# 10183308/popsift

Hardware: AMD Instinct MI355X
Metric: Mpix/s SIFT extract on 1920x1080 (keypoints+descriptors) (higher is better)
Workload: dtype f32; 1 GPU; 1920x1080 u8 grayscale, default popsift::Config (2x upscale, 9 octaves, 3 levels, PopSift mode, loop descriptor, RootSift); distinct_images_per_gpu=16, contexts_per_gpu=3, images_per_launch=16

## Files before the change

### popsift_amd/csrc/ctx.hip

```cpp
#include <hip/hip_runtime.h>

#include <algorithm>
#include <cmath>
#include <cstdarg>
#include <cstddef>
#include <cstdio>
#include <cstdlib>
#include <cstring>
#include <new>
#include <vector>

#include "devfeatures.h"
#include "ext_list.h"
#include "kernels.h"
#include "sift_types.h"
#include "trace.h"

using namespace popsift_hip;

namespace {

constexpr int PITCH_ALIGN = 64;
constexpr int PROFILE_REPS = 4;

// ... 30 lines not shown
struct ImageSlot {
    DevBuf<char> input;
    void*        h_input = nullptr;
    size_t       h_input_cap = 0;
    DevBuf<float>       arena;
    DevBuf<InitExt>     iext;
    DevBuf<InitExt>     iext2;
    DevBuf<FilterState> fstate;
    DevBuf<int>         fhist;
    DevBuf<InitExt>     otmp;
    DevBuf<int>         orows;
    DevBuf<float>       sresp_in, sresp;
    DevBuf<StrongState> sstate;
    DevBuf<int>         schunk;
    DevBuf<Ext>         ext;
    DevBuf<float, PS_ORI_NBINS> ohist;
    DevBuf<popsift_hip_feature> feats;
    DevBuf<float, 128> desc;
    DevBuf<int>        map;
    DevBuf<float2>     rot;
    DevBuf<DescRec>    drec;
    DevBuf<int2>       cand;
    DevBuf<int>        partial;
    DevBuf<int>        ovf;
    bool               sized = false;
    DevBuf<popsift_hip_feature> alt_feats;
    DevBuf<float, 128>          alt_desc;
    bool moved = false;
    DevBuf<uint8_t, 128> desc_u8;
    bool u8_read = false;
    DevBuf<popsift_hip_frame>   frames;
    popsift_hip_frame*          h_frames = nullptr;
    DevBuf<int>                 fcounts, perm, inv;
    DevBuf<popsift_hip_feature> lfeats;
    int n_frames = 0;
    DevBuf<uint8_t> mask;
    void*           h_mask = nullptr;
    size_t          h_mask_cap = 0;

    size_t desc_cap() const { return std::min({desc.cap, map.cap, rot.cap, drec.cap}); }

    void release()
    {
        auto each = [](auto&... b) { ((void)b.release(), ...); };
        each(input, arena, iext, iext2, fstate, fhist, otmp, orows, sresp_in, sresp, sstate, schunk, ext, ohist, feats, desc, map, rot, drec, cand, partial, ovf, alt_feats,
             alt_desc, desc_u8, frames, fcounts, perm, inv, lfeats, mask);
        if (h_input) (void)hipHostFree(h_input);
        if (h_mask) (void)hipHostFree(h_mask);
        if (h_frames) (void)hipHostFree(h_frames);
    }
};

struct popsift_hip_ctx {
    int                device = 0;
    popsift_hip_params p{};
    int                levels = 3, L = 6;
    GaussRows<POPSIFT_HIP_MAX_LEVELS> tab{};
    GaussRows<POPSIFT_HIP_MAX_LEVELS> abs0{};
    float*             d_abs0 = nullptr;
    int                direct_path = 0;
// ... 238 lines not shown
    return hipMalloc(p, bytes);
}

template <class T, size_t PER>
int grow(popsift_hip_ctx* c, DevBuf<T, PER>& b, size_t need)
{
    if (need <= b.cap) return 0;
    HIP_TRY(c, b.release());
    HIP_TRY(c, ctx_malloc(c, (void**)&b.p, need * PER * sizeof(T)));
    b.cap = need;
    return 0;
}

void refresh_caps(popsift_hip_ctx* c)
{
    size_t cand = 1 << 30, desc = 1 << 30, hist = (size_t)1 << 40;
    for (int k = 0; k < c->nb; k++) {
        const ImageSlot& s = c->slot[k];
        cand = std::min(cand, s.cand.cap);
        desc = std::min(desc, s.desc_cap());
        hist = std::min(hist, s.ohist.cap);
        Slot& v = c->bd.s[k];
        v.arena = s.arena.p;
        v.ct = c->d_ct + k;
        v.cand = s.cand.p;
        v.ovf = s.ovf.p;
        v.iext = s.iext.p;
        v.iext2 = s.iext2.p;
        v.fstate = s.fstate.p;
        v.fhist = s.fhist.p;
        v.ohist = s.ohist.p;
        v.ext = s.ext.p;
        v.partial = s.partial.p;
        v.map = s.map.p;
        v.rot = s.rot.p;
        v.drec = s.drec.p;
        v.feats = s.feats.p;
        v.desc = s.desc.p;
    }
    c->cand_cap = (int)cand;
    c->desc_cap = (int)desc;
    c->ohist_cap = hist;
}

int slot_desc_cap(popsift_hip_ctx* c, ImageSlot& s, size_t need)
{
    if (need <= s.desc_cap()) return 0;
    HIP_TRY(c, s.desc.release());
    HIP_TRY(c, s.map.release());
    HIP_TRY(c, s.rot.release());
    HIP_TRY(c, s.drec.release());
    if (int rc = grow(c, s.desc, need)) return rc;
    if (int rc = grow(c, s.map, need)) return rc;
    if (int rc = grow(c, s.rot, need)) return rc;
    return grow(c, s.drec, need);
}

// ... 21 lines not shown
        c->frozen_octaves = plan.n_oct;

        c->in_w = c->in_h = 0;
        c->have_image = false;
        c->pd.n_oct = 0;
        c->ext_cap = 0;
        for (int k = 0; k < PS_MAX_BATCH; k++) c->slot[k].sized = false;

        pd = plan;
    } else {
        const OctDesc& last = pd.o[pd.n_oct - 1];
        total = pd.dog_fly ? (size_t)pd.o[0].dog_off + (size_t)pd.o[0].plane_stride
                           : (size_t)last.dog_off + (size_t)last.plane_stride * (size_t)(c->L - 1);
    }
    const size_t need_ext = (size_t)pd.n_oct * (size_t)c->sc.max_extrema;
    for (int k = 0; k < nb; k++) {
        ImageSlot& s = c->slot[k];
        if (s.sized) continue;
        if (int rc = grow(c, s.arena, total)) return rc;
        if (int rc = grow(c, s.iext, need_ext)) return rc;
        if (int rc = grow(c, s.ext, need_ext)) return rc;
        if (int rc = grow(c, s.feats, need_ext)) return rc;
        if (c->sc.filter_max > 0) {
            if (int rc = grow(c, s.iext2, need_ext)) return rc;
            if (int rc = grow(c, s.fstate, 1)) return rc;
            if (int rc = grow(c, s.fhist, filter_hist_bytes(c->sc.grid_size) / sizeof(int))) return rc;
        }
        if (c->p.feature_order == POPSIFT_HIP_ORDER_RASTER) {
            if (int rc = grow(c, s.otmp, need_ext)) return rc;
            if (int rc = grow(c, s.orows, order_rows(pd))) return rc;
        }
        if (int rc = grow(c, s.partial, (need_ext / scan_chunk() + 2) * scan_partials_per_chunk())) return rc;
        const int desc0 = c->desc_cap_init > 0 ? c->desc_cap_init
                                               : std::max(2 * c->sc.max_extrema, c->sc.max_extrema + c->sc.max_extrema / 4);
        if (int rc = slot_desc_cap(c, s, std::max(desc0, c->desc_cap))) return rc;
        int cand0 = std::max(c->cand_cap_init, DET_SUBQ);
        if (!c->cand_cap_user) {
            double px = 0;
            for (int o = 0; o < pd.n_oct; o++) px += (double)pd.o[o].w * pd.o[o].h;
            cand0 = std::max(cand0, (int)std::min(px / 8.0, 64.0 * 1024 * 1024));
        }
        if (int rc = grow(c, s.cand, std::max(cand0, c->cand_cap))) return rc;
        if (int rc = grow(c, s.ohist, std::max(c->ohist_cap_init > 0 ? (size_t)c->ohist_cap_init
                                                                      : std::min(need_ext, (size_t)2 * c->sc.max_extrema),
                                               c->slot[0].sized ? c->ohist_cap : (size_t)0)))
            return rc;
        if (int rc = grow(c, s.ovf, (size_t)pd.total_tiles + 1)) return rc;
        s.sized = true;
    }
    c->ext_cap = need_ext;
    if (!same) {
        *c->h_pd = pd;
        HIP_TRY(c, hipMemcpyAsync(c->d_pd, c->h_pd, sizeof(PyrDesc), hipMemcpyHostToDevice, c->stream));
        c->pd = pd;
        c->in_w = w;
        c->in_h = h;
        c->rep.num_octaves = pd.n_oct;
        c->rep.base_w = bw;
        c->rep.base_h = bh;
        double px = 0;
        for (int o = 0; o < pd.n_oct; o++) px += (double)pd.o[o].w * pd.o[o].h;
// ... 316 lines not shown
    }
    return launch_strongest(c->pd, c->d_pd, c->sc, c->batch_keep, sb, c->nb, c->stream);
}

int enqueue_descriptor_stages(popsift_hip_ctx* c, const BatchDesc& lb, bool filtered, bool with_ori, const FrameBatch* fb)
{
    const bool stages = (c->profile == 2);
    auto       mark = [&](int k) -> hipError_t { return stages ? hipEventRecord(c->ev_stage[k], c->stream) : hipSuccess; };
    HIP_TRY(c, mark(POPSIFT_HIP_STAGE_ORIENTATION));
    if (with_ori) {
        HIP_TRY(c, launch_orientation(c->d_pd, c->bd, c->nb, c->sc, filtered, (int)c->ohist_cap, c->kp_waves, c->stream));
        SYNC_CHK(c, "k_orientation");
    }
    HIP_TRY(c, mark(POPSIFT_HIP_STAGE_SCAN));
    const int n_chunks = std::max((int)(((size_t)c->pd.n_oct * c->sc.max_extrema + scan_chunk() - 1) / scan_chunk()), 1);
    if (with_ori)
        HIP_TRY(c, launch_scan(c->d_pd, lb, c->nb, c->sc, filtered, (int)c->ohist_cap, n_chunks, c->desc_cap, c->stream));
    else
        HIP_TRY(c, launch_scan_apply(c->d_pd, lb, c->nb, c->sc, n_chunks, c->desc_cap, c->stream));
    SYNC_CHK(c, "k_scan_local / k_scan_apply");
    HIP_TRY(c, mark(POPSIFT_HIP_STAGE_DESCRIPTOR));
    HIP_TRY(c, launch_descriptors(c->d_pd, c->bd, c->nb, c->sc, c->desc_cap, c->kp_waves, c->stream));
    SYNC_CHK(c, "descriptor kernel");
    if (fb) {
        HIP_TRY(c, launch_frame_out(c->bd, *fb, c->nb, c->desc_cap, c->frames_max, c->stream));
        SYNC_CHK(c, "k_frame_out");
    }
    HIP_TRY(c, mark(POPSIFT_HIP_STAGE_COUNT));
    HIP_TRY(c, hipMemcpyAsync(c->h_ct, c->d_ct, sizeof(Counters) * (size_t)c->nb, hipMemcpyDeviceToHost, c->stream));
    return 0;
}

int enqueue_keypoint_stages(popsift_hip_ctx* c, bool counters_cleared = false)
{
    POPSIFT_RANGE("popsift_hip: keypoint stages");
// ... 218 lines not shown
            ext_max = std::max(ext_max, ext_sum);
        }
        const bool desc_short = ori_max > c->desc_cap;
        const bool cand_short = qmax > c->cand_cap / DET_SUBQ;
        const bool hist_short = (size_t)ext_max > c->ohist_cap && !c->ori_given;
        if (!desc_short && !cand_short && !hist_short) {
            fits = true;
            break;
        }
        if (desc_short)
            if (int rc = ensure_cap(c, [&](ImageSlot& s) { return slot_desc_cap(c, s, ori_max + ori_max / 8 + 1024); }))
                return rc;
        if (cand_short)
            if (int rc = ensure_cap(c, [&](ImageSlot& s) { return grow(c, s.cand, DET_SUBQ * (qmax + qmax / 8 + 64)); }))
                return rc;
        if (hist_short) {
            const size_t need = (size_t)ext_max + (size_t)ext_max / 8 + 1024;
            if (int rc = ensure_cap(c, [&](ImageSlot& s) { return grow(c, s.ohist, need); })) return rc;
        }
        if (int rc = c->describe ? enqueue_describe_stages(c) : enqueue_keypoint_stages(c)) return rc;
        HIP_TRY(c, hipEventRecord(c->ev_end, c->stream));
        rerun = true;
    }
    if (!fits) return fail(c, POPSIFT_HIP_ERR_DEVICE, "the keypoint buffers still do not fit after 8 grow-and-rerun rounds");
    popsift_hip_report& r = c->rep;
    for (int k = 0; k < c->nb; k++) {
        c->n_feat[k] = c->describe ? c->slot[k].n_frames : c->h_ct[k].ext_total;
        c->n_desc[k] = std::min(c->h_ct[k].ori_total, c->desc_cap);
    }
    Counters& h0 = c->h_ct[0];
    int       next = h0.ori_total;
    for (int o = PS_MAX_OCT - 1; o >= 0; o--) {
        if (h0.ext_ct[o] > 0) {
            h0.ori_ct[o] = next - h0.ori_ps[o];
// ... 804 lines not shown
```

### popsift_amd/csrc/kernels.h

```cpp
#pragma once
#include <hip/hip_runtime.h>

#include <algorithm>

#include "sift_types.h"

namespace popsift_hip {

struct Taps {
    float g[PS_GA];
};

struct BlurArgs {
    int64_t src_off;
    int64_t dst_off;
    int64_t dog_off;
    int     w, h, pitch;
    int     tiles_x, tiles_y;
    int     in_w, in_h, in_pitch;
    float   shift;
    int     fast2x;
    Taps    taps;
    int64_t next0_off;
    int     next_pitch;
// ... 56 lines not shown
hipError_t launch_blur_octaves(const BlurArgs& base, int level, const PyrDesc* d_pd, const PyrDesc& pd, const BatchDesc& bd,
                               int nb, int halo, hipStream_t s);
hipError_t launch_blur_level0_sep(const BlurArgs& a, const Taps& vt, const BatchDesc& bd, int nb, int halo, int is_f32,
                                  hipStream_t s);
int        scale_tile_h();

hipError_t launch_dog_plane(float* dog, const float* upper, const float* lower, size_t n, hipStream_t s);
int        extrema_units(int w, int h);
hipError_t launch_extrema(const PyrDesc& pd, const PyrDesc* d_pd, const BatchDesc& bd, int nb, const SiftConsts& sc, int cand_cap,
                          bool filtered, hipStream_t s, hipEvent_t mid, const MaskArgs* ma);

hipError_t launch_orientation(const PyrDesc* d_pd, const BatchDesc& bd, int nb, const SiftConsts& sc, bool filtered, int hist_cap,
                              int blocks, hipStream_t s);
int        scan_chunk();
int        scan_partials_per_chunk();
hipError_t launch_scan(const PyrDesc* d_pd, const BatchDesc& bd, int nb, const SiftConsts& sc, bool filtered, int hist_cap,
                       int n_chunks, int desc_cap, hipStream_t s);
hipError_t launch_descriptors(const PyrDesc* d_pd, const BatchDesc& bd, int nb, const SiftConsts& sc, int desc_cap, int blocks,
                              hipStream_t s);

hipError_t launch_desc_modes(const PyrDesc* d_pd, const BatchDesc& bd, int nb, const SiftConsts& sc, int desc_cap, int blocks,
                             hipStream_t s);

hipError_t launch_scan_apply(const PyrDesc* d_pd, const BatchDesc& bd, int nb, const SiftConsts& sc, int n_chunks, int desc_cap,
                             hipStream_t s);

constexpr int FRAME_CHUNK = 256;
int        frame_chunks(int n_max);
hipError_t launch_frame_count(const PyrDesc* d_pd, const FrameBatch& fb, int nb, const SiftConsts& sc, int given, int n_max,
                              hipStream_t s);
hipError_t launch_frame_place(const PyrDesc* d_pd, const BatchDesc& bd, const FrameBatch& fb, int nb, const SiftConsts& sc,
                              int given, int n_max, hipStream_t s);
// ... 41 lines not shown
```

### popsift_amd/csrc/keypoint.hip

```cpp
#include <hip/hip_runtime.h>

#include "ext_list.h"
#include "kernels.h"
#include "keypoint_dev.h"
#include "sift_types.h"

namespace popsift_hip {
namespace {

constexpr float ORI_WINFACTOR = 1.5f;

struct Taps {
    const char* row;
    const char* dn;
    const char* up;
    __device__ __forceinline__ Taps(const float* layer, int pitch)
        : row((const char*)layer), dn((const char*)(layer + pitch)), up((const char*)(layer - pitch)) {}
    __device__ __forceinline__ void load_b(unsigned int b, float& xp, float& xm, float& yp, float& ym) const
    {
        xp = *(const float*)(row + (size_t)b + 4);
        xm = *(const float*)(row + (size_t)b - 4);
        yp = *(const float*)(dn + (size_t)b);
        ym = *(const float*)(up + (size_t)b);
    }
// ... 38 lines not shown
    const float d = (fabsf(x) + 1e-18f) + mod;
    const float t = y * __builtin_amdgcn_rcpf(d);
    const float s = t * t;
    float       p = fmaf(-0.02984253503382206f, s, 0.13406537473201752f);
    p = fmaf(p, s, -0.2964776158332825f);
    p = fmaf(p, s, 0.4928465187549591f);
    p = fmaf(p, s, -0.8470170497894287f);
    p = fmaf(p, s, 2.5464210510253906f);
    const float th = t * p;
    const float sg = copysignf(scale, x);
    return fmaf(th, sg, fmaf(-2.0f, sg, k0));
}

typedef __attribute__((address_space(3))) fix64 lds_fix64;
typedef __attribute__((address_space(3))) unsigned int lds_u32;
typedef __attribute__((address_space(3))) short lds_i16;
typedef __attribute__((address_space(3))) unsigned long long lds_u64;

#ifndef KP_NW
#define KP_NW 1
#endif
constexpr int ORI_COPIES = 4;

__global__ __launch_bounds__(64 * KP_NW) void k_orientation(const PyrDesc* __restrict__ pdp, BatchDesc bd, SiftConsts sc,
                                                     int filtered, int hist_cap)
{
    const float* __restrict__   arena = bd.s[blockIdx.y].arena;
    Counters* __restrict__      ct = bd.s[blockIdx.y].ct;
    const InitExt* __restrict__ iext = filtered ? bd.s[blockIdx.y].iext2 : bd.s[blockIdx.y].iext;
    float* __restrict__         ohist = bd.s[blockIdx.y].ohist;
    const int n_oct = pdp->n_oct, L = pdp->L;
    constexpr int    NB = PS_ORI_NBINS + 10;
    __shared__ fix64 s_hist[KP_NW][ORI_COPIES][NB];
    const int        wave = threadIdx.x >> 6, lane = threadIdx.x & 63;
    fix64*           hall = &s_hist[wave][0][0];
    fix64*           hist = s_hist[wave][lane & (ORI_COPIES - 1)];

    __shared__ int ps[PS_MAX_OCT + 1];
    const int total = min(ext_prefix(ps, ct, sc.max_extrema, n_oct), hist_cap);

    for (XcdSlice sl = xcd_slice<KP_NW>(); sl.more(total); sl.s += sl.step) {
        const int g = sl.index();
        if (g >= total) continue;
        const int o = uniform(ext_octave(ps, n_oct, g));
        const InitExt  ie = iext[(size_t)o * sc.max_extrema + (g - uniform(ps[o]))];
        const OctDesc* od = &pdp->o[o];
        const int      w = uniform(od->w), h = uniform(od->h), pitch = uniform(od->pitch);
        const int      lvl = uniform(min(max(ie.lpos, 0), L - 1));
        const float*   layer = arena + uniform64(od->data_off + lvl * od->plane_stride);

        for (int k = lane; k < ORI_COPIES * NB; k += 64) hall[k] = 0ull;
        wave_lds_sync();

        const float x = uniformf(ie.xpos), y = uniformf(ie.ypos), sig = uniformf(ie.sigma);
        const float sigw = ORI_WINFACTOR * sig;
        const int   rad = (int)roundf(3.0f * sigw);
        const float factor2 = (-0.5f / (sigw * sigw)) * 1.4426950408889634f;
        const int   sq_thres = rad * rad;
// ... 53 lines not shown
            bin(xb, yb, b0 - b1, b2 - b3, true);
        }
        if (t == 2) {
            coord(min(i + 64, loops - 1), xb, yb, ob);
            taps.load_b(ob, b0, b1, b2, b3);
        }
        if (t > 0) bin(xa, ya, a0 - a1, a2 - a3, i < loops);
        if (t == 2) bin(xb, yb, b0 - b1, b2 - b3, i + 64 < loops);
        wave_lds_sync();

        if (lane < PS_ORI_NBINS) {
            fix64 acc = 0ull;
#pragma unroll
            for (int k = 0; k < ORI_COPIES; k++)
                acc += hall[k * NB + lane] + (lane < NB - PS_ORI_NBINS ? hall[k * NB + PS_ORI_NBINS + lane] : 0ull);
            ohist[(size_t)g * PS_ORI_NBINS + lane] = from_fix(acc);
        }
        wave_lds_sync();
    }
}

__device__ __forceinline__ float quad_from_prev(float v)
{
    return __int_as_float(__builtin_amdgcn_update_dpp(0, __float_as_int(v), 0x93, 0xf, 0xf, false));
}
__device__ __forceinline__ float quad_from_next(float v)
{
    return __int_as_float(__builtin_amdgcn_update_dpp(0, __float_as_int(v), 0x39, 0xf, 0xf, false));
}
template <int CTRL>
__device__ __forceinline__ int quad_xchg(int v)
{
    return __builtin_amdgcn_update_dpp(0, v, CTRL, 0xf, 0xf, false);
}
__device__ __forceinline__ float div3(float x)
{
    const float r = 0.333333343267440796f;
    const float q = x * r;
    return fmaf(fmaf(-3.0f, q, x), r, q);
}

__device__ __forceinline__ int ori_peaks_quad(const float* __restrict__ hsrc, int j, bool have, float* angle_out)
{
    constexpr int N = PS_ORI_NBINS, M = N / 4;
    float         h[M], t[M];
#pragma unroll
    for (int b = 0; b < M; b++) h[b] = have ? hsrc[M * j + b] : 0.0f;
#pragma unroll
    for (int pass = 0; pass < 3; pass++) {
        {
            const float lft = quad_from_prev(h[M - 1]), rgt = quad_from_next(h[0]);
#pragma unroll
            for (int b = 0; b < M; b++) t[b] = div3(((b == 0 ? lft : h[b - 1]) + h[b]) + (b == M - 1 ? rgt : h[b + 1]));
        }
        {
            const float lft = quad_from_prev(t[M - 1]), rgt = quad_from_next(t[0]);
#pragma unroll
            for (int b = 0; b < M; b++) h[b] = div3(((b == 0 ? lft : t[b - 1]) + t[b]) + (b == M - 1 ? rgt : t[b + 1]));
        }
    }
    float refined[M], yval[M];
    {
        const float lft = quad_from_prev(h[M - 1]), rgt = quad_from_next(h[0]);
#pragma unroll
        for (int b = 0; b < M; b++) {
            const int   bin = M * j + b;
            const int   prev = (bin == 0) ? N - 1 : bin - 1;
            const float hp = (b == 0) ? lft : h[b - 1], hv = h[b], hn = (b == M - 1) ? rgt : h[b + 1];
            bool        predicate = hv > fmaxf(hp, hn);
            const float num = predicate ? 3.0f * hp - 4.0f * hv + 1.0f * hn : 0.0f;
            const float denB = predicate ? 2.0f * (hp - 2.0f * hv + hn) : 1.0f;
            const float newbin = num / denB;
            predicate = (predicate && newbin >= 0.0f && newbin <= 2.0f);
            refined[b] = predicate ? prev + newbin : -1.0f;
            yval[b] = predicate ? -(num * num) / (4.0f * denB) + hp : -INFINITY;
        }
    }
    unsigned int used = 0u;
    float        best0 = 0.0f;
    int          angles = 0;
#pragma unroll
    for (int k = 0; k < POPSIFT_HIP_ORI_MAX; k++) {
        float bv = 0.0f, br = -1.0f;
        int   bi = -1;
#pragma unroll
        for (int b = 0; b < M; b++) {
            const bool take = !((used >> b) & 1u) && (bi < 0 || yval[b] > bv);
            bv = take ? yval[b] : bv;
            br = take ? refined[b] : br;
            bi = take ? M * j + b : bi;
        }
        {
            const float ov = __int_as_float(quad_xchg<0xB1>(__float_as_int(bv))), orf = __int_as_float(quad_xchg<0xB1>(__float_as_int(br)));
            const int   oi = quad_xchg<0xB1>(bi);
            const bool  take = ov > bv || (ov == bv && oi < bi);
            bv = take ? ov : bv;
            br = take ? orf : br;
            bi = take ? oi : bi;
        }
        {
            const float ov = __int_as_float(quad_xchg<0x4E>(__float_as_int(bv))), orf = __int_as_float(quad_xchg<0x4E>(__float_as_int(br)));
            const int   oi = quad_xchg<0x4E>(bi);
            const bool  take = ov > bv || (ov == bv && oi < bi);
            bv = take ? ov : bv;
            br = take ? orf : br;
            bi = take ? oi : bi;
        }
        const int mine = bi - M * j;
        if (mine >= 0 && mine < M) used |= 1u << mine;
        if (k == 0) best0 = bv;
        if (bv >= 0.8f * best0) {
            float chosen_bin = br;
            if (chosen_bin >= N) chosen_bin -= N;
            angle_out[k] = fmaf(F_PI2 * chosen_bin, 1.0f / N, -F_PI);
            angles = k + 1;
        } else {
            angle_out[k] = 0.0f;
        }
    }
    return angles;
}

__device__ __forceinline__ DescRec make_desc_rec(const PyrDesc* __restrict__ pdp, const Ext& e, float angle, float cos_t, float sin_t)
{
    DescRec        r;
    const OctDesc* od = &pdp->o[e.octave];
    const int      lvl = min(max(e.lpos, 0), pdp->L - 1);
    const long long off = od->data_off + lvl * od->plane_stride;
    const float    x = e.xpos, y = e.ypos;
    const float    SBP = fabsf(DESC_MAGNIFY * e.sigma);
    const float    cell_px = (2.83f * SBP + 1.0f) * (2.83f * SBP + 1.0f);
    const int      fbits = min(max(31 - (int)ceilf(log2f(361.0f * cell_px)), 2), 14);
    const float    csbp = cos_t * SBP, ssbp = sin_t * SBP;
    const float    bsz = fabsf(csbp) + fabsf(ssbp);
    const float    ext_r = 2.5f * bsz;
// ... 8 lines not shown
    r.ang_bins = angle * (4.0f / F_PI);
    if (!(fabsf(r.ang_bins) <= 16.0f)) r.ang_bins = (float)remainder((double)angle * (4.0 / 3.14159265358979323846), 8.0);
    r.inv_c = (fabsf(r.crsbp) > 1e-20f) ? __builtin_amdgcn_rcpf(r.crsbp) : 0.0f;
    r.inv_s = (fabsf(r.srsbp) > 1e-20f) ? __builtin_amdgcn_rcpf(r.srsbp) : 0.0f;
    r.xymin = ((unsigned int)xmin & 0xffffu) | ((unsigned int)ymin << 16);
    r.xymax = ((unsigned int)xmax & 0xffffu) | ((unsigned int)ymax << 16);
    r.off_lo = (unsigned int)((unsigned long long)off & 0xffffffffull);
    r.off_hi = (unsigned int)((unsigned long long)off >> 32);
    r.misc = (unsigned int)od->pitch | ((unsigned int)fbits << 16) | ((SBP != 0.0f) ? (1u << 24) : 0u);
    return r;
}


constexpr int SCAN_ITEMS = 1;
constexpr int SCAN_CHUNK = 256 * SCAN_ITEMS;
constexpr int SCAN_LT = 256;
constexpr int SCAN_LCHUNK = SCAN_LT / 4;
constexpr int SCAN_SUB = SCAN_CHUNK / SCAN_LCHUNK;

__global__ __launch_bounds__(SCAN_LT) void k_scan_local(const PyrDesc* __restrict__ pdp, SiftConsts sc, BatchDesc bd,
                                                     int filtered, int hist_cap)
{
    const Counters* __restrict__ ct = bd.s[blockIdx.y].ct;
    const InitExt* __restrict__  iext = filtered ? bd.s[blockIdx.y].iext2 : bd.s[blockIdx.y].iext;
    const float* __restrict__    ohist = bd.s[blockIdx.y].ohist;
    Ext* __restrict__            ext = bd.s[blockIdx.y].ext;
    int* __restrict__            partial = bd.s[blockIdx.y].partial;
    static_assert(SCAN_CHUNK % SCAN_LCHUNK == 0 && SCAN_LT % 64 == 0, "four lanes per extremum, whole waves");
    __shared__ int s_wsum[SCAN_LT / 64];
    __shared__ int s_ps[PS_MAX_OCT + 1];
    const int      n_oct = pdp->n_oct;
    const int total = ext_prefix(s_ps, ct, sc.max_extrema, n_oct);
    const int tid = threadIdx.x;
    const int j = tid & 3;
    for (int chunk = blockIdx.x; chunk * SCAN_LCHUNK < total; chunk += gridDim.x) {
    const int  base = chunk * SCAN_LCHUNK;
    const int  g = base + (tid >> 2);
    const bool valid = g < total;
    const int  gc = min(g, total - 1);
    const int     o = ext_octave(s_ps, n_oct, gc);
    const InitExt ie = iext[(size_t)o * sc.max_extrema + (gc - s_ps[o])];
    Ext           e;
    e.xpos = ie.xpos;
    e.ypos = ie.ypos;
    e.lpos = ie.lpos;
    e.sigma = ie.sigma;
    e.octave = o;
    e.idx_ori = 0;
    const bool have = gc < hist_cap;
    const int  n = ori_peaks_quad(ohist + (size_t)min(gc, max(hist_cap - 1, 0)) * PS_ORI_NBINS, j, have, e.orientation);
    e.num_ori = have ? n : 0;
    if (!have)
        for (int q = 0; q < POPSIFT_HIP_ORI_MAX; q++) e.orientation[q] = 0.0f;
    const int self = (valid && j == 0) ? e.num_ori : 0;

    const WgScan scan = wg_scan<SCAN_LT / 64>(self, s_wsum);
    if (valid && j == 0) {
        e.idx_ori = scan.excl;
        ext[g] = e;
    }
    if (tid == SCAN_LT - 1) partial[chunk] = scan.excl + self;
    __syncthreads();
    }
}

__global__ __launch_bounds__(256) void k_scan_apply(const PyrDesc* __restrict__ pdp, SiftConsts sc, BatchDesc bd,
                                                    int with_drec, int desc_cap)
{
    Counters* __restrict__            ct = bd.s[blockIdx.y].ct;
    Ext* __restrict__                 ext = bd.s[blockIdx.y].ext;
    const int* __restrict__           partial = bd.s[blockIdx.y].partial;
    int* __restrict__                 map = bd.s[blockIdx.y].map;
    float2* __restrict__              rot = bd.s[blockIdx.y].rot;
    DescRec* __restrict__             drec = with_drec ? bd.s[blockIdx.y].drec : nullptr;
    popsift_hip_feature* __restrict__ feats = bd.s[blockIdx.y].feats;
    __shared__ int s_red[4];
    __shared__ int s_ps[PS_MAX_OCT + 1];
    const int      n_oct = pdp->n_oct;
    const int      tid = threadIdx.x, lane = tid & 63, wave = tid >> 6;
    const int total = ext_prefix(s_ps, ct, sc.max_extrema, n_oct);
    const int nb = (total + SCAN_CHUNK - 1) / SCAN_CHUNK;
    if (nb == 0 && blockIdx.x == 0 && tid == 0) {
        ct->ori_total = 0;
        ct->ext_total = 0;
        for (int o = 0; o < PS_MAX_OCT; o++) {
            ct->ext_ct[o] = 0;
            ct->ext_ps[o] = 0;
        }
    }
    for (int chunk = blockIdx.x; chunk < nb; chunk += gridDim.x) {
    const int base = chunk * SCAN_CHUNK;

    int acc = 0;
    for (int b = tid; b < chunk * SCAN_SUB; b += 256) acc += partial[b];
    acc = wave_sum(acc);
    if (lane == 0) s_red[wave] = acc;
    __syncthreads();
    const int chunk_offset = s_red[0] + s_red[1] + s_red[2] + s_red[3];
    int offset = chunk_offset;
    for (int k = 0; k < (tid * SCAN_ITEMS) / SCAN_LCHUNK; k++) offset += partial[chunk * SCAN_SUB + k];

    const int g0 = base + tid * SCAN_ITEMS;
#pragma unroll
    for (int k = 0; k < SCAN_ITEMS; k++) {
        const int g = g0 + k;
        if (g < total) {
            Ext       e = ext[g];
            const int idx = e.idx_ori + offset;
            const int n = e.num_ori;
            ext[g].idx_ori = idx;
            popsift_hip_feature f;
            const float         scl = powf(2.0f, (float)(e.octave - sc.up_fac_int));
            f.debug_octave = e.octave;
            f.xpos = e.xpos * scl;
            f.ypos = e.ypos * scl;
// ... 332 lines not shown
            const float rn = scalbnf(__builtin_amdgcn_rsqf(sq), sc.norm_multi);
            v0 = v0 * rn;
            v1 = v1 * rn;
        }
        desc[(size_t)d * 128 + lane] = v0;
        desc[(size_t)d * 128 + 64 + lane] = v1;
        wave_lds_sync();
    }
}

}

hipError_t launch_orientation(const PyrDesc* pd, const BatchDesc& bd, int nb, const SiftConsts& sc, bool filtered, int hist_cap,
                              int blocks, hipStream_t s)
{
    hipLaunchKernelGGL(k_orientation, dim3(blocks / KP_NW, nb), dim3(64 * KP_NW), 0, s, pd, bd, sc, filtered ? 1 : 0, hist_cap);
    return hipGetLastError();
}

hipError_t launch_scan(const PyrDesc* pd, const BatchDesc& bd, int nb, const SiftConsts& sc, bool filtered, int hist_cap,
                       int n_chunks, int desc_cap, hipStream_t s)
{
    hipLaunchKernelGGL(k_scan_local, dim3(std::min(n_chunks * SCAN_SUB, 512 * SCAN_SUB), nb), dim3(SCAN_LT), 0, s, pd, sc, bd,
                       filtered ? 1 : 0, hist_cap);
    return launch_scan_apply(pd, bd, nb, sc, n_chunks, desc_cap, s);
}

hipError_t launch_scan_apply(const PyrDesc* pd, const BatchDesc& bd, int nb, const SiftConsts& sc, int n_chunks, int desc_cap,
                             hipStream_t s)
{
    hipLaunchKernelGGL(k_scan_apply, dim3(std::min(n_chunks, 1024), nb), dim3(256), 0, s, pd, sc, bd,
                       sc.desc_mode == POPSIFT_HIP_DESC_LOOP ? 1 : 0, desc_cap);
    return hipGetLastError();
}

int scan_chunk() { return SCAN_CHUNK; }
int scan_partials_per_chunk() { return SCAN_SUB; }

hipError_t launch_descriptors(const PyrDesc* pd, const BatchDesc& bd, int nb, const SiftConsts& sc, int desc_cap, int blocks,
                              hipStream_t s)
// ... 10 lines not shown
```

### popsift_amd/csrc/keypoint_dev.h

```cpp
#pragma once
#include <hip/hip_runtime.h>

#include "wave_dev.h"

namespace popsift_hip {

constexpr float F_PI = 3.14159265358979323846f;
constexpr float F_PI2 = 2.0f * 3.14159265358979323846f;
constexpr float DESC_MAGNIFY = 3.0f;

typedef unsigned long long fix64;
__device__ __forceinline__ float from_fix(fix64 v) { return (float)((double)v * (1.0 / 1048576.0)); }

__device__ __forceinline__ void wave_lds_sync()
{
    __builtin_amdgcn_fence(__ATOMIC_SEQ_CST, "wavefront");
    __builtin_amdgcn_wave_barrier();
}

__device__ __forceinline__ float wave_allsum(float v)
{
#define PS_DPP_ADD(CTRL) v += __int_as_float(__builtin_amdgcn_update_dpp(0, __float_as_int(v), CTRL, 0xf, 0xf, false))
    PS_DPP_ADD(0xB1);
    PS_DPP_ADD(0x4E);
// ... 3 lines not shown
    const float r0 = __int_as_float(__builtin_amdgcn_readlane(__float_as_int(v), 0));
    const float r1 = __int_as_float(__builtin_amdgcn_readlane(__float_as_int(v), 16));
    const float r2 = __int_as_float(__builtin_amdgcn_readlane(__float_as_int(v), 32));
    const float r3 = __int_as_float(__builtin_amdgcn_readlane(__float_as_int(v), 48));
    return (r0 + r1) + (r2 + r3);
}

__device__ __forceinline__ float plane_at(const float* pl, int idx)
{
    return *(const float*)((const char*)pl + (size_t)((unsigned int)idx * 4u));
}

#ifndef KP_CHUNK
#define KP_CHUNK 256
#endif
struct XcdSlice {
    int x, s, step;
    __device__ __forceinline__ int index() const { return ((s / KP_CHUNK) * 8 + x) * KP_CHUNK + (s % KP_CHUNK); }
    __device__ __forceinline__ bool more(int total) const { return (s / KP_CHUNK) * 8 * KP_CHUNK < total; }
};
template <int NW>
__device__ __forceinline__ XcdSlice xcd_slice()
{
    XcdSlice sl;
    sl.x = blockIdx.x & 7;
    sl.s = (int)(blockIdx.x >> 3) * NW + uniform((int)(threadIdx.x >> 6));
    sl.step = (int)(gridDim.x >> 3) * NW;
    return sl;
}

__device__ __forceinline__ float div_nr(float a, float b)
{
    const float r = __builtin_amdgcn_rcpf(b);
    const float q = a * r;
    return fmaf(fmaf(-b, q, a), r, q);
}
__device__ __forceinline__ float atan2_acc(float y, float x)
{
    const float ax = fabsf(x), ay = fabsf(y);
// ... 16 lines not shown
```

### popsift_amd/csrc/sift_types.h

```cpp
#pragma once
#include <stdint.h>

#include <hip/hip_vector_types.h>

#include "../../include/popsift_hip.h"

#define PS_MAX_OCT POPSIFT_HIP_MAX_OCTAVES
#define PS_MAX_PLANES (POPSIFT_HIP_MAX_LEVELS + 3)
#define PS_GA POPSIFT_HIP_GAUSS_ALIGN
#define PS_ORI_NBINS 36

struct OctDesc {
    float*  data;
    float*  dog;
    int64_t data_off;
    int64_t dog_off;
    int64_t plane_stride;
    int     w, h, pitch;
    int     tile_begin;
};

struct PyrDesc {
    int     n_oct;
    int     levels;
// ... 62 lines not shown
};
#define DET_SUBQ 64

#define PS_MAX_BATCH POPSIFT_HIP_MAX_BATCH
struct FilterState;
struct Slot {
    float*               arena;
    Counters*            ct;
    const void*          input;
    int2*                cand;
    int*                 ovf;
    InitExt*             iext;
    InitExt*             iext2;
    FilterState*         fstate;
    int*                 fhist;
    float*               ohist;
    Ext*                 ext;
    int*                 partial;
    int*                 map;
    float2*              rot;
    DescRec*             drec;
    popsift_hip_feature* feats;
    float*               desc;
};
struct BatchDesc {
    Slot s[PS_MAX_BATCH];
};

#define FILTER_MAX_CELLS 4096
struct FilterState {
    int                active;
// ... 81 lines not shown
```

Before: 4011 Mpix/s.

## Fuse orientation peak finding and local scan into the orientation kernel

The orientation kernel now processes groups of 16 extrema per wave, keeps their histograms in LDS instead of writing them to a global ohist buffer, then runs the quad-lane peak search and a wave-level scan in the same kernel, writing Ext records and per-group partials. The separate k_scan_local kernel and the per-slot ohist allocation are removed, and scan_apply gains a vectorised partial sum plus a one-wave sub-chunk prefix in place of a serial loop. This saves a global round trip of histograms and one kernel launch. In exchange it uses more LDS per block and sets a launch-bounds occupancy hint, and the orientation grid is resized. The work per wave is also coarser, which may hurt load balance.

```diff
diff --git a/popsift_amd/csrc/ctx.hip b/popsift_amd/csrc/ctx.hip
--- a/popsift_amd/csrc/ctx.hip
+++ b/popsift_amd/csrc/ctx.hip
@@ -68,7 +68,6 @@
     DevBuf<StrongState> sstate;
     DevBuf<int>         schunk;
     DevBuf<Ext>         ext;
-    DevBuf<float, PS_ORI_NBINS> ohist;
     DevBuf<popsift_hip_feature> feats;
     DevBuf<float, 128> desc;
     DevBuf<int>        map;
@@ -97,7 +96,7 @@
     void release()
     {
         auto each = [](auto&... b) { ((void)b.release(), ...); };
-        each(input, arena, iext, iext2, fstate, fhist, otmp, orows, sresp_in, sresp, sstate, schunk, ext, ohist, feats, desc, map, rot, drec, cand, partial, ovf, alt_feats,
+        each(input, arena, iext, iext2, fstate, fhist, otmp, orows, sresp_in, sresp, sstate, schunk, ext, feats, desc, map, rot, drec, cand, partial, ovf, alt_feats,
              alt_desc, desc_u8, frames, fcounts, perm, inv, lfeats, mask);
         if (h_input) (void)hipHostFree(h_input);
         if (h_mask) (void)hipHostFree(h_mask);
@@ -366,12 +365,11 @@
 
 void refresh_caps(popsift_hip_ctx* c)
 {
-    size_t cand = 1 << 30, desc = 1 << 30, hist = (size_t)1 << 40;
+    size_t cand = 1 << 30, desc = 1 << 30;
     for (int k = 0; k < c->nb; k++) {
         const ImageSlot& s = c->slot[k];
         cand = std::min(cand, s.cand.cap);
         desc = std::min(desc, s.desc_cap());
-        hist = std::min(hist, s.ohist.cap);
         Slot& v = c->bd.s[k];
         v.arena = s.arena.p;
         v.ct = c->d_ct + k;
@@ -381,7 +379,6 @@
         v.iext2 = s.iext2.p;
         v.fstate = s.fstate.p;
         v.fhist = s.fhist.p;
-        v.ohist = s.ohist.p;
         v.ext = s.ext.p;
         v.partial = s.partial.p;
         v.map = s.map.p;
@@ -392,7 +389,6 @@
     }
     c->cand_cap = (int)cand;
     c->desc_cap = (int)desc;
-    c->ohist_cap = hist;
 }
 
 int slot_desc_cap(popsift_hip_ctx* c, ImageSlot& s, size_t need)
@@ -444,6 +440,8 @@
                            : (size_t)last.dog_off + (size_t)last.plane_stride * (size_t)(c->L - 1);
     }
     const size_t need_ext = (size_t)pd.n_oct * (size_t)c->sc.max_extrema;
+    c->ohist_cap = std::max(c->ohist_cap, c->ohist_cap_init > 0 ? (size_t)c->ohist_cap_init
+                                                                 : std::min(need_ext, (size_t)2 * c->sc.max_extrema));
     for (int k = 0; k < nb; k++) {
         ImageSlot& s = c->slot[k];
         if (s.sized) continue;
@@ -471,10 +469,6 @@
             cand0 = std::max(cand0, (int)std::min(px / 8.0, 64.0 * 1024 * 1024));
         }
         if (int rc = grow(c, s.cand, std::max(cand0, c->cand_cap))) return rc;
-        if (int rc = grow(c, s.ohist, std::max(c->ohist_cap_init > 0 ? (size_t)c->ohist_cap_init
-                                                                      : std::min(need_ext, (size_t)2 * c->sc.max_extrema),
-                                               c->slot[0].sized ? c->ohist_cap : (size_t)0)))
-            return rc;
         if (int rc = grow(c, s.ovf, (size_t)pd.total_tiles + 1)) return rc;
         s.sized = true;
     }
@@ -821,11 +815,8 @@
     }
     HIP_TRY(c, mark(POPSIFT_HIP_STAGE_SCAN));
     const int n_chunks = std::max((int)(((size_t)c->pd.n_oct * c->sc.max_extrema + scan_chunk() - 1) / scan_chunk()), 1);
-    if (with_ori)
-        HIP_TRY(c, launch_scan(c->d_pd, lb, c->nb, c->sc, filtered, (int)c->ohist_cap, n_chunks, c->desc_cap, c->stream));
-    else
-        HIP_TRY(c, launch_scan_apply(c->d_pd, lb, c->nb, c->sc, n_chunks, c->desc_cap, c->stream));
-    SYNC_CHK(c, "k_scan_local / k_scan_apply");
+    HIP_TRY(c, launch_scan_apply(c->d_pd, lb, c->nb, c->sc, n_chunks, c->desc_cap, c->stream));
+    SYNC_CHK(c, "k_scan_apply");
     HIP_TRY(c, mark(POPSIFT_HIP_STAGE_DESCRIPTOR));
     HIP_TRY(c, launch_descriptors(c->d_pd, c->bd, c->nb, c->sc, c->desc_cap, c->kp_waves, c->stream));
     SYNC_CHK(c, "descriptor kernel");
@@ -1074,10 +1065,7 @@
         if (cand_short)
             if (int rc = ensure_cap(c, [&](ImageSlot& s) { return grow(c, s.cand, DET_SUBQ * (qmax + qmax / 8 + 64)); }))
                 return rc;
-        if (hist_short) {
-            const size_t need = (size_t)ext_max + (size_t)ext_max / 8 + 1024;
-            if (int rc = ensure_cap(c, [&](ImageSlot& s) { return grow(c, s.ohist, need); })) return rc;
-        }
+        if (hist_short) c->ohist_cap = std::max(c->ohist_cap, (size_t)ext_max + (size_t)ext_max / 8 + 1024);
         if (int rc = c->describe ? enqueue_describe_stages(c) : enqueue_keypoint_stages(c)) return rc;
         HIP_TRY(c, hipEventRecord(c->ev_end, c->stream));
         rerun = true;
diff --git a/popsift_amd/csrc/kernels.h b/popsift_amd/csrc/kernels.h
--- a/popsift_amd/csrc/kernels.h
+++ b/popsift_amd/csrc/kernels.h
@@ -94,8 +94,6 @@
                               int blocks, hipStream_t s);
 int        scan_chunk();
 int        scan_partials_per_chunk();
-hipError_t launch_scan(const PyrDesc* d_pd, const BatchDesc& bd, int nb, const SiftConsts& sc, bool filtered, int hist_cap,
-                       int n_chunks, int desc_cap, hipStream_t s);
 hipError_t launch_descriptors(const PyrDesc* d_pd, const BatchDesc& bd, int nb, const SiftConsts& sc, int desc_cap, int blocks,
                               hipStream_t s);
 
diff --git a/popsift_amd/csrc/keypoint.hip b/popsift_amd/csrc/keypoint.hip
--- a/popsift_amd/csrc/keypoint.hip
+++ b/popsift_amd/csrc/keypoint.hip
@@ -76,6 +76,7 @@
 
 typedef __attribute__((address_space(3))) fix64 lds_fix64;
 typedef __attribute__((address_space(3))) unsigned int lds_u32;
+typedef __attribute__((address_space(3))) float lds_f32;
 typedef __attribute__((address_space(3))) short lds_i16;
 typedef __attribute__((address_space(3))) unsigned long long lds_u64;
 
@@ -84,13 +85,118 @@
 #endif
 constexpr int ORI_COPIES = 4;
 
-__global__ __launch_bounds__(64 * KP_NW) void k_orientation(const PyrDesc* __restrict__ pdp, BatchDesc bd, SiftConsts sc,
-                                                     int filtered, int hist_cap)
+__device__ __forceinline__ float div3(float x)
+{
+    const float r = 0.333333343267440796f;
+    const float q = x * r;
+    return fmaf(fmaf(-3.0f, q, x), r, q);
+}
+
+__device__ __forceinline__ float quad_from_prev(float v)
+{
+    return __int_as_float(__builtin_amdgcn_update_dpp(0, __float_as_int(v), 0x93, 0xf, 0xf, false));
+}
+__device__ __forceinline__ float quad_from_next(float v)
+{
+    return __int_as_float(__builtin_amdgcn_update_dpp(0, __float_as_int(v), 0x39, 0xf, 0xf, false));
+}
+template <int CTRL>
+__device__ __forceinline__ int quad_xchg(int v)
+{
+    return __builtin_amdgcn_update_dpp(0, v, CTRL, 0xf, 0xf, false);
+}
+
+__device__ __forceinline__ int ori_peaks_quad(const lds_f32* __restrict__ hsrc, int j, bool have, float* angle_out)
+{
+    constexpr int N = PS_ORI_NBINS, M = N / 4;
+    float         h[M], t[M];
+#pragma unroll
+    for (int b = 0; b < M; b++) h[b] = have ? hsrc[M * j + b] : 0.0f;
+#pragma unroll
+    for (int pass = 0; pass < 3; pass++) {
+        {
+            const float lft = quad_from_prev(h[M - 1]), rgt = quad_from_next(h[0]);
+#pragma unroll
+            for (int b = 0; b < M; b++) t[b] = div3(((b == 0 ? lft : h[b - 1]) + h[b]) + (b == M - 1 ? rgt : h[b + 1]));
+        }
+        {
+            const float lft = quad_from_prev(t[M - 1]), rgt = quad_from_next(t[0]);
+#pragma unroll
+            for (int b = 0; b < M; b++) h[b] = div3(((b == 0 ? lft : t[b - 1]) + t[b]) + (b == M - 1 ? rgt : t[b + 1]));
+        }
+    }
+    float refined[M], yval[M];
+    {
+        const float lft = quad_from_prev(h[M - 1]), rgt = quad_from_next(h[0]);
+#pragma unroll
+        for (int b = 0; b < M; b++) {
+            const int   bin = M * j + b;
+            const int   prev = (bin == 0) ? N - 1 : bin - 1;
+            const float hp = (b == 0) ? lft : h[b - 1], hv = h[b], hn = (b == M - 1) ? rgt : h[b + 1];
+            bool        predicate = hv > fmaxf(hp, hn);
+            const float num = predicate ? 3.0f * hp - 4.0f * hv + 1.0f * hn : 0.0f;
+            const float denB = predicate ? 2.0f * (hp - 2.0f * hv + hn) : 1.0f;
+            const float newbin = num / denB;
+            predicate = (predicate && newbin >= 0.0f && newbin <= 2.0f);
+            refined[b] = predicate ? prev + newbin : -1.0f;
+            yval[b] = predicate ? -(num * num) / (4.0f * denB) + hp : -INFINITY;
+        }
+    }
+    unsigned int used = 0u;
+    float        best0 = 0.0f;
+    int          angles = 0;
+#pragma unroll
+    for (int k = 0; k < POPSIFT_HIP_ORI_MAX; k++) {
+        float bv = 0.0f, br = -1.0f;
+        int   bi = -1;
+#pragma unroll
+        for (int b = 0; b < M; b++) {
+            const bool take = !((used >> b) & 1u) && (bi < 0 || yval[b] > bv);
+            bv = take ? yval[b] : bv;
+            br = take ? refined[b] : br;
+            bi = take ? M * j + b : bi;
+        }
+        {
+            const float ov = __int_as_float(quad_xchg<0xB1>(__float_as_int(bv))), orf = __int_as_float(quad_xchg<0xB1>(__float_as_int(br)));
+            const int   oi = quad_xchg<0xB1>(bi);
+            const bool  take = ov > bv || (ov == bv && oi < bi);
+            bv = take ? ov : bv;
+            br = take ? orf : br;
+            bi = take ? oi : bi;
+        }
+        {
+            const float ov = __int_as_float(quad_xchg<0x4E>(__float_as_int(bv))), orf = __int_as_float(quad_xchg<0x4E>(__float_as_int(br)));
+            const int   oi = quad_xchg<0x4E>(bi);
+            const bool  take = ov > bv || (ov == bv && oi < bi);
+            bv = take ? ov : bv;
+            br = take ? orf : br;
+            bi = take ? oi : bi;
+        }
+        const int mine = bi - M * j;
+        if (mine >= 0 && mine < M) used |= 1u << mine;
+        if (k == 0) best0 = bv;
+        if (bv >= 0.8f * best0) {
+            float chosen_bin = br;
+            if (chosen_bin >= N) chosen_bin -= N;
+            angle_out[k] = fmaf(F_PI2 * chosen_bin, 1.0f / N, -F_PI);
+            angles = k + 1;
+        } else {
+            angle_out[k] = 0.0f;
+        }
+    }
+    return angles;
+}
+
+constexpr int SCAN_LCHUNK = KP_GROUP;
+
+__global__ __launch_bounds__(64 * KP_NW, 8) void k_orientation(const PyrDesc* __restrict__ pdp, BatchDesc bd, SiftConsts sc,
+                                                        int filtered, int hist_cap)
 {
     const float* __restrict__   arena = bd.s[blockIdx.y].arena;
     Counters* __restrict__      ct = bd.s[blockIdx.y].ct;
     const InitExt* __restrict__ iext = filtered ? bd.s[blockIdx.y].iext2 : bd.s[blockIdx.y].iext;
-    float* __restrict__         ohist = bd.s[blockIdx.y].ohist;
+    Ext* __restrict__           ext = bd.s[blockIdx.y].ext;
+    int* __restrict__           partial = bd.s[blockIdx.y].partial;
     const int n_oct = pdp->n_oct, L = pdp->L;
     constexpr int    NB = PS_ORI_NBINS + 10;
     __shared__ fix64 s_hist[KP_NW][ORI_COPIES][NB];
@@ -98,12 +204,18 @@
     fix64*           hall = &s_hist[wave][0][0];
     fix64*           hist = s_hist[wave][lane & (ORI_COPIES - 1)];
 
+    __shared__ float s_stage[KP_NW][KP_GROUP][PS_ORI_NBINS];
+    static_assert(KP_GROUP * 4 == 64, "four lanes per extremum of a group");
+    static_assert(sizeof(s_hist) / KP_NW + sizeof(s_stage) / KP_NW + 64 <= 5120, "32 waves per CU share 160 KiB");
+
     __shared__ int ps[PS_MAX_OCT + 1];
-    const int total = min(ext_prefix(ps, ct, sc.max_extrema, n_oct), hist_cap);
-
-    for (XcdSlice sl = xcd_slice<KP_NW>(); sl.more(total); sl.s += sl.step) {
-        const int g = sl.index();
-        if (g >= total) continue;
+    const int total = ext_prefix(ps, ct, sc.max_extrema, n_oct);
+
+    for (XcdSliceOf<KP_GROUP> sl = xcd_slice<KP_NW, KP_GROUP>(); sl.more(total); sl.s += sl.step) {
+        const int g0 = uniform(sl.index());
+        if (g0 >= total) continue;
+        const int g_end = min(min(g0 + KP_GROUP, total), hist_cap);
+        for (int g = g0; g < g_end; g++) {
         const int o = uniform(ext_octave(ps, n_oct, g));
         const InitExt  ie = iext[(size_t)o * sc.max_extrema + (g - uniform(ps[o]))];
         const OctDesc* od = &pdp->o[o];
@@ -187,111 +299,39 @@
 #pragma unroll
             for (int k = 0; k < ORI_COPIES; k++)
                 acc += hall[k * NB + lane] + (lane < NB - PS_ORI_NBINS ? hall[k * NB + PS_ORI_NBINS + lane] : 0ull);
-            ohist[(size_t)g * PS_ORI_NBINS + lane] = from_fix(acc);
+            s_stage[wave][g - g0][lane] = from_fix(acc);
         }
         wave_lds_sync();
-    }
-}
-
-__device__ __forceinline__ float quad_from_prev(float v)
-{
-    return __int_as_float(__builtin_amdgcn_update_dpp(0, __float_as_int(v), 0x93, 0xf, 0xf, false));
-}
-__device__ __forceinline__ float quad_from_next(float v)
-{
-    return __int_as_float(__builtin_amdgcn_update_dpp(0, __float_as_int(v), 0x39, 0xf, 0xf, false));
-}
-template <int CTRL>
-__device__ __forceinline__ int quad_xchg(int v)
-{
-    return __builtin_amdgcn_update_dpp(0, v, CTRL, 0xf, 0xf, false);
-}
-__device__ __forceinline__ float div3(float x)
-{
-    const float r = 0.333333343267440796f;
-    const float q = x * r;
-    return fmaf(fmaf(-3.0f, q, x), r, q);
-}
-
-__device__ __forceinline__ int ori_peaks_quad(const float* __restrict__ hsrc, int j, bool have, float* angle_out)
-{
-    constexpr int N = PS_ORI_NBINS, M = N / 4;
-    float         h[M], t[M];
-#pragma unroll
-    for (int b = 0; b < M; b++) h[b] = have ? hsrc[M * j + b] : 0.0f;
-#pragma unroll
-    for (int pass = 0; pass < 3; pass++) {
+        }
+
         {
-            const float lft = quad_from_prev(h[M - 1]), rgt = quad_from_next(h[0]);
-#pragma unroll
-            for (int b = 0; b < M; b++) t[b] = div3(((b == 0 ? lft : h[b - 1]) + h[b]) + (b == M - 1 ? rgt : h[b + 1]));
-        }
-        {
-            const float lft = quad_from_prev(t[M - 1]), rgt = quad_from_next(t[0]);
-#pragma unroll
-            for (int b = 0; b < M; b++) h[b] = div3(((b == 0 ? lft : t[b - 1]) + t[b]) + (b == M - 1 ? rgt : t[b + 1]));
-        }
-    }
-    float refined[M], yval[M];
-    {
-        const float lft = quad_from_prev(h[M - 1]), rgt = quad_from_next(h[0]);
-#pragma unroll
-        for (int b = 0; b < M; b++) {
-            const int   bin = M * j + b;
-            const int   prev = (bin == 0) ? N - 1 : bin - 1;
-            const float hp = (b == 0) ? lft : h[b - 1], hv = h[b], hn = (b == M - 1) ? rgt : h[b + 1];
-            bool        predicate = hv > fmaxf(hp, hn);
-            const float num = predicate ? 3.0f * hp - 4.0f * hv + 1.0f * hn : 0.0f;
-            const float denB = predicate ? 2.0f * (hp - 2.0f * hv + hn) : 1.0f;
-            const float newbin = num / denB;
-            predicate = (predicate && newbin >= 0.0f && newbin <= 2.0f);
-            refined[b] = predicate ? prev + newbin : -1.0f;
-            yval[b] = predicate ? -(num * num) / (4.0f * denB) + hp : -INFINITY;
-        }
-    }
-    unsigned int used = 0u;
-    float        best0 = 0.0f;
-    int          angles = 0;
-#pragma unroll
-    for (int k = 0; k < POPSIFT_HIP_ORI_MAX; k++) {
-        float bv = 0.0f, br = -1.0f;
-        int   bi = -1;
-#pragma unroll
-        for (int b = 0; b < M; b++) {
-            const bool take = !((used >> b) & 1u) && (bi < 0 || yval[b] > bv);
-            bv = take ? yval[b] : bv;
-            br = take ? refined[b] : br;
-            bi = take ? M * j + b : bi;
-        }
-        {
-            const float ov = __int_as_float(quad_xchg<0xB1>(__float_as_int(bv))), orf = __int_as_float(quad_xchg<0xB1>(__float_as_int(br)));
-            const int   oi = quad_xchg<0xB1>(bi);
-            const bool  take = ov > bv || (ov == bv && oi < bi);
-            bv = take ? ov : bv;
-            br = take ? orf : br;
-            bi = take ? oi : bi;
-        }
-        {
-            const float ov = __int_as_float(quad_xchg<0x4E>(__float_as_int(bv))), orf = __int_as_float(quad_xchg<0x4E>(__float_as_int(br)));
-            const int   oi = quad_xchg<0x4E>(bi);
-            const bool  take = ov > bv || (ov == bv && oi < bi);
-            bv = take ? ov : bv;
-            br = take ? orf : br;
-            bi = take ? oi : bi;
-        }
-        const int mine = bi - M * j;
-        if (mine >= 0 && mine < M) used |= 1u << mine;
-        if (k == 0) best0 = bv;
-        if (bv >= 0.8f * best0) {
-            float chosen_bin = br;
-            if (chosen_bin >= N) chosen_bin -= N;
-            angle_out[k] = fmaf(F_PI2 * chosen_bin, 1.0f / N, -F_PI);
-            angles = k + 1;
-        } else {
-            angle_out[k] = 0.0f;
-        }
-    }
-    return angles;
+            const int  j = lane & 3;
+            const int  g = g0 + (lane >> 2);
+            const bool valid = g < total;
+            const int  gc = min(g, total - 1);
+            const int     o = ext_octave(ps, n_oct, gc);
+            const InitExt ie = iext[(size_t)o * sc.max_extrema + (gc - ps[o])];
+            Ext           e;
+            e.xpos = ie.xpos;
+            e.ypos = ie.ypos;
+            e.lpos = ie.lpos;
+            e.sigma = ie.sigma;
+            e.octave = o;
+            const bool have = gc < hist_cap;
+            const int  n = ori_peaks_quad((const lds_f32*)&s_stage[wave][gc - g0][0], j, have, e.orientation);
+            e.num_ori = have ? n : 0;
+            if (!have)
+                for (int q = 0; q < POPSIFT_HIP_ORI_MAX; q++) e.orientation[q] = 0.0f;
+            const int self = (valid && j == 0) ? e.num_ori : 0;
+            const int incl = wave_incl_scan(self);
+            if (valid && j == 0) {
+                e.idx_ori = incl - self;
+                ext[g] = e;
+            }
+            if (lane == 63) partial[g0 / SCAN_LCHUNK] = incl;
+        }
+        wave_lds_sync();
+    }
 }
 
 __device__ __forceinline__ DescRec make_desc_rec(const PyrDesc* __restrict__ pdp, const Ext& e, float angle, float cos_t, float sin_t)
@@ -330,55 +370,8 @@
 
 constexpr int SCAN_ITEMS = 1;
 constexpr int SCAN_CHUNK = 256 * SCAN_ITEMS;
-constexpr int SCAN_LT = 256;
-constexpr int SCAN_LCHUNK = SCAN_LT / 4;
 constexpr int SCAN_SUB = SCAN_CHUNK / SCAN_LCHUNK;
-
-__global__ __launch_bounds__(SCAN_LT) void k_scan_local(const PyrDesc* __restrict__ pdp, SiftConsts sc, BatchDesc bd,
-                                                     int filtered, int hist_cap)
-{
-    const Counters* __restrict__ ct = bd.s[blockIdx.y].ct;
-    const InitExt* __restrict__  iext = filtered ? bd.s[blockIdx.y].iext2 : bd.s[blockIdx.y].iext;
-    const float* __restrict__    ohist = bd.s[blockIdx.y].ohist;
-    Ext* __restrict__            ext = bd.s[blockIdx.y].ext;
-    int* __restrict__            partial = bd.s[blockIdx.y].partial;
-    static_assert(SCAN_CHUNK % SCAN_LCHUNK == 0 && SCAN_LT % 64 == 0, "four lanes per extremum, whole waves");
-    __shared__ int s_wsum[SCAN_LT / 64];
-    __shared__ int s_ps[PS_MAX_OCT + 1];
-    const int      n_oct = pdp->n_oct;
-    const int total = ext_prefix(s_ps, ct, sc.max_extrema, n_oct);
-    const int tid = threadIdx.x;
-    const int j = tid & 3;
-    for (int chunk = blockIdx.x; chunk * SCAN_LCHUNK < total; chunk += gridDim.x) {
-    const int  base = chunk * SCAN_LCHUNK;
-    const int  g = base + (tid >> 2);
-    const bool valid = g < total;
-    const int  gc = min(g, total - 1);
-    const int     o = ext_octave(s_ps, n_oct, gc);
-    const InitExt ie = iext[(size_t)o * sc.max_extrema + (gc - s_ps[o])];
-    Ext           e;
-    e.xpos = ie.xpos;
-    e.ypos = ie.ypos;
-    e.lpos = ie.lpos;
-    e.sigma = ie.sigma;
-    e.octave = o;
-    e.idx_ori = 0;
-    const bool have = gc < hist_cap;
-    const int  n = ori_peaks_quad(ohist + (size_t)min(gc, max(hist_cap - 1, 0)) * PS_ORI_NBINS, j, have, e.orientation);
-    e.num_ori = have ? n : 0;
-    if (!have)
-        for (int q = 0; q < POPSIFT_HIP_ORI_MAX; q++) e.orientation[q] = 0.0f;
-    const int self = (valid && j == 0) ? e.num_ori : 0;
-
-    const WgScan scan = wg_scan<SCAN_LT / 64>(self, s_wsum);
-    if (valid && j == 0) {
-        e.idx_ori = scan.excl;
-        ext[g] = e;
-    }
-    if (tid == SCAN_LT - 1) partial[chunk] = scan.excl + self;
-    __syncthreads();
-    }
-}
+static_assert(SCAN_CHUNK % SCAN_LCHUNK == 0 && SCAN_SUB <= 64, "whole groups per chunk, one lane of a wave per group");
 
 __global__ __launch_bounds__(256) void k_scan_apply(const PyrDesc* __restrict__ pdp, SiftConsts sc, BatchDesc bd,
                                                     int with_drec, int desc_cap)
@@ -391,6 +384,7 @@
     DescRec* __restrict__             drec = with_drec ? bd.s[blockIdx.y].drec : nullptr;
     popsift_hip_feature* __restrict__ feats = bd.s[blockIdx.y].feats;
     __shared__ int s_red[4];
+    __shared__ int s_sub[SCAN_SUB];
     __shared__ int s_ps[PS_MAX_OCT + 1];
     const int      n_oct = pdp->n_oct;
     const int      tid = threadIdx.x, lane = tid & 63, wave = tid >> 6;
@@ -407,14 +401,22 @@
     for (int chunk = blockIdx.x; chunk < nb; chunk += gridDim.x) {
     const int base = chunk * SCAN_CHUNK;
 
+    static_assert(SCAN_SUB % 4 == 0, "16-byte loads of the partials");
     int acc = 0;
-    for (int b = tid; b < chunk * SCAN_SUB; b += 256) acc += partial[b];
+    for (int b = tid; b < chunk * (SCAN_SUB / 4); b += 256) {
+        const int4 v = reinterpret_cast<const int4*>(partial)[b];
+        acc += (v.x + v.y) + (v.z + v.w);
+    }
     acc = wave_sum(acc);
     if (lane == 0) s_red[wave] = acc;
+    if (wave == 0) {
+        const int v = (lane < SCAN_SUB) ? partial[chunk * SCAN_SUB + lane] : 0;
+        const int incl = wave_incl_scan(v);
+        if (lane < SCAN_SUB) s_sub[lane] = incl - v;
+    }
     __syncthreads();
     const int chunk_offset = s_red[0] + s_red[1] + s_red[2] + s_red[3];
-    int offset = chunk_offset;
-    for (int k = 0; k < (tid * SCAN_ITEMS) / SCAN_LCHUNK; k++) offset += partial[chunk * SCAN_SUB + k];
+    const int offset = chunk_offset + s_sub[(tid * SCAN_ITEMS) / SCAN_LCHUNK];
 
     const int g0 = base + tid * SCAN_ITEMS;
 #pragma unroll
@@ -777,16 +779,9 @@
 hipError_t launch_orientation(const PyrDesc* pd, const BatchDesc& bd, int nb, const SiftConsts& sc, bool filtered, int hist_cap,
                               int blocks, hipStream_t s)
 {
-    hipLaunchKernelGGL(k_orientation, dim3(blocks / KP_NW, nb), dim3(64 * KP_NW), 0, s, pd, bd, sc, filtered ? 1 : 0, hist_cap);
+    const int waves = std::max(blocks / 8 / (8 * KP_NW) * (8 * KP_NW), 8 * KP_NW);
+    hipLaunchKernelGGL(k_orientation, dim3(waves / KP_NW, nb), dim3(64 * KP_NW), 0, s, pd, bd, sc, filtered ? 1 : 0, hist_cap);
     return hipGetLastError();
-}
-
-hipError_t launch_scan(const PyrDesc* pd, const BatchDesc& bd, int nb, const SiftConsts& sc, bool filtered, int hist_cap,
-                       int n_chunks, int desc_cap, hipStream_t s)
-{
-    hipLaunchKernelGGL(k_scan_local, dim3(std::min(n_chunks * SCAN_SUB, 512 * SCAN_SUB), nb), dim3(SCAN_LT), 0, s, pd, sc, bd,
-                       filtered ? 1 : 0, hist_cap);
-    return launch_scan_apply(pd, bd, nb, sc, n_chunks, desc_cap, s);
 }
 
 hipError_t launch_scan_apply(const PyrDesc* pd, const BatchDesc& bd, int nb, const SiftConsts& sc, int n_chunks, int desc_cap,
diff --git a/popsift_amd/csrc/keypoint_dev.h b/popsift_amd/csrc/keypoint_dev.h
--- a/popsift_amd/csrc/keypoint_dev.h
+++ b/popsift_amd/csrc/keypoint_dev.h
@@ -41,15 +41,20 @@
 #ifndef KP_CHUNK
 #define KP_CHUNK 256
 #endif
-struct XcdSlice {
+constexpr int KP_GROUP = 16;
+template <int UNIT>
+struct XcdSliceOf {
+    static constexpr int PER_CHUNK = KP_CHUNK / UNIT;
+    static_assert(KP_CHUNK % UNIT == 0, "whole groups per chunk");
     int x, s, step;
-    __device__ __forceinline__ int index() const { return ((s / KP_CHUNK) * 8 + x) * KP_CHUNK + (s % KP_CHUNK); }
-    __device__ __forceinline__ bool more(int total) const { return (s / KP_CHUNK) * 8 * KP_CHUNK < total; }
+    __device__ __forceinline__ int index() const { return ((s / PER_CHUNK) * 8 + x) * KP_CHUNK + (s % PER_CHUNK) * UNIT; }
+    __device__ __forceinline__ bool more(int total) const { return (s / PER_CHUNK) * 8 * KP_CHUNK < total; }
 };
-template <int NW>
-__device__ __forceinline__ XcdSlice xcd_slice()
+typedef XcdSliceOf<1> XcdSlice;
+template <int NW, int UNIT = 1>
+__device__ __forceinline__ XcdSliceOf<UNIT> xcd_slice()
 {
-    XcdSlice sl;
+    XcdSliceOf<UNIT> sl;
     sl.x = blockIdx.x & 7;
     sl.s = (int)(blockIdx.x >> 3) * NW + uniform((int)(threadIdx.x >> 6));
     sl.step = (int)(gridDim.x >> 3) * NW;
diff --git a/popsift_amd/csrc/sift_types.h b/popsift_amd/csrc/sift_types.h
--- a/popsift_amd/csrc/sift_types.h
+++ b/popsift_amd/csrc/sift_types.h
@@ -100,7 +100,6 @@
     InitExt*             iext2;
     FilterState*         fstate;
     int*                 fhist;
-    float*               ohist;
     Ext*                 ext;
     int*                 partial;
     int*                 map;
```

New measurement: 4057 Mpix/s, median of 6. 1.01x the previous value.
